# Tanveer81/ReVisionLLM

Hardware: AMD Instinct MI355X
Metric: video-segments/sec (whole node), stage-2 100-seg recursion, Vicuna-7B (higher is better)
Workload: dtype fp16

## Files before the change

revisionllm_amd/csrc/attention.hip:

```cpp
#include "kernels.h"

#ifndef ATTN_PAIR_Q32
#define ATTN_PAIR_Q32 0
#endif

namespace {

template <int DH, bool SPLIT, bool PAD, bool QS = false>
__device__ __forceinline__ void attn_body(const AttnArgs& a, int bx, int h, int b, [[maybe_unused]] float* merge = nullptr) {
    constexpr int NC = DH / 32, ND = DH / 16;
    const int lane = threadIdx.x & 63;
    const int wave = __builtin_amdgcn_readfirstlane(threadIdx.x >> 6);
    const int fr = lane & 15, g = lane >> 4;
    const int q0 = SPLIT ? bx * 16 : bx * 64 + wave * 16;
    if (q0 >= a.Lq) return;
    const int kb_ = b / a.kv_div;
    const int Lk = a.row_pos ? a.row_pos[b] + 1 : a.Lk;
    if (Lk <= 0 || (a.row_pos && Lk > a.Lk)) return;
    const int q_pos0 = a.row_pos ? Lk - a.Lq : a.q_pos0;

    const op16_t* qp = (const op16_t*)a.q + (int64_t)b * a.q_bs + (int64_t)min(q0 + fr, a.Lq - 1) * a.q_rs + h * DH + g * 8;
    op16x8 qf[NC];
#pragma unroll
    for (int c = 0; c < NC; ++c) qf[c] = *(const op16x8*)(qp + c * 32);
    op16x8 ql[QS ? NC : 1];
    if constexpr (QS) {
#pragma unroll
        for (int c = 0; c < NC; ++c) ql[c] = *(const op16x8*)(qp + a.q_lo + c * 32);
    }

    const op16_t* kbase = (const op16_t*)a.k + (int64_t)kb_ * a.k_bs + (int64_t)h * a.k_hs + g * 8;
    const op16_t* vbase = (const op16_t*)a.vt + (int64_t)kb_ * a.vt_bs + (int64_t)h * a.vt_hs + (int64_t)fr * a.vt_ds + g * a.vt_ks;
    int share_len = 0;
// ... 491 lines not shown
        const float alpha = __expf(m_run - m_use);
        float psum = 0.f;
        float p[8];
#pragma unroll
        for (int t = 0; t < 2; ++t)
#pragma unroll
            for (int r = 0; r < 4; ++r) {
                const float e = __expf(s[t][r] - m_use);
                p[t * 4 + r] = e;
                psum += e;
            }
        l_run = l_run * alpha + psum;
        m_run = m_new;
        union { op16x8 v; uint32_t u[4]; } pf;
#pragma unroll
        for (int j = 0; j < 4; ++j) pf.u[j] = pack_op16x2_bounded(p[2 * j], p[2 * j + 1]);
        if (__builtin_amdgcn_ballot_w64(alpha != 1.0f) != 0) {
#pragma unroll
            for (int dt = 0; dt < ND; ++dt) o[dt] *= alpha;
        }
#pragma unroll
        for (int dt = 0; dt < ND; ++dt) o[dt] = rv_mfma16(vf[dt], pf.v, o[dt]);
    }
    l_run += __shfl_xor(l_run, 16, 64);
    l_run += __shfl_xor(l_run, 32, 64);
    if (q0 + fr >= a.Lq) return;
    const float inv = 1.0f / l_run;
    op16_t* op = (op16_t*)a.out + (int64_t)b * a.o_bs + (int64_t)(q0 + fr) * a.o_rs + h * DH + g * 4;
#pragma unroll
    for (int dt = 0; dt < ND; ++dt)
        *(u32x2*)(op + dt * 16) = pack_op16x4(f32x4{o[dt][0] * inv, o[dt][1] * inv, o[dt][2] * inv, o[dt][3] * inv});
}

__device__ __forceinline__ bool attn_map(int tiles, int H, int pairs, int& bx, int& h, int& b) {
    const int id = blockIdx.x, j = id >> 3;
    const int pr = (j / tiles) * 8 + (id & 7);
    if (pr >= pairs) return false;
    bx = j % tiles;
    h = pr % H;
    b = pr / H;
    return true;
}
__host__ inline unsigned attn_grid(int tiles, int pairs) { return (unsigned)(tiles * ((pairs + 7) / 8) * 8); }

template <int DH, bool SPLIT, bool QS = false>
__global__ __launch_bounds__(256, DH <= 128 ? 3 : 1) void attn_kernel(AttnArgs a, int tiles) {
    int bx, h, b;
    if (!attn_map(tiles, a.H, a.H * a.B, bx, h, b)) return;
    __shared__ __attribute__((aligned(16))) float merge[SPLIT ? 4 * 16 * (DH + 4) + 2 * 4 * 16 : 4];
    if constexpr (QS) attn_body<DH, SPLIT, false, true>(a, bx, h, b, merge);
    else if (a.key_pad) attn_body<DH, SPLIT, true>(a, bx, h, b, merge);
    else attn_body<DH, SPLIT, false>(a, bx, h, b, merge);
}

template <int DH>
__global__ __launch_bounds__(256, 2) void attn_kernel_lds(AttnArgs a, int tiles) {
    __shared__ __attribute__((aligned(16))) char smem[2 * (2 * (DH / 32) + DH / 16) * 1024];
    int bx, h, b;
    if (!attn_map(tiles, a.H, a.H * a.B, bx, h, b)) return;
    attn_body_lds<DH>(a, bx, h, b, smem);
}

template <int DH, bool QS = false>
__global__ __launch_bounds__(256, 3) void attn_kernel_pair(AttnArgs a, AttnArgs b, int tiles, AttnGroups gr) {
    int bx, h, z;
    const int per = a.B + b.B;
// ... 44 lines not shown
}

__device__ __forceinline__ void attn_mixed_problem(AttnArgs& p, const AttnMixed& mx, int z, int& b) {
    int g = 0;
    for (int i = 1; i < mx.G; ++i) g += z >= mx.first[i] ? 1 : 0;
    const QkvGroup e = mx.gt[g];
    const int zl = z - mx.first[g], hasp = e.P0 > 0 ? 1 : 0;
    const bool prefix = hasp && zl == 0;
    const int64_t row0 = prefix ? e.base : e.base + e.P0;
    p.q = (const op16_t*)p.q + row0 * p.q_rs;
    p.out = (op16_t*)p.out + row0 * p.o_rs;
    p.k = (const op16_t*)p.k + (int64_t)e.row * p.k_bs;
    p.vt = (const op16_t*)p.vt + (int64_t)e.row * p.vt_bs;
    if (prefix) { p.B = 1; p.Lq = p.Lk = e.P0; p.q_pos0 = 0; p.q_bs = (int64_t)e.P0 * p.q_rs; p.o_bs = (int64_t)e.P0 * p.o_rs; b = 0; }
    else { p.B = e.B; p.Lq = e.S; p.Lk = e.P0 + e.S; p.q_pos0 = e.P0; p.q_bs = (int64_t)e.S * p.q_rs; p.o_bs = (int64_t)e.S * p.o_rs; b = zl - hasp; }
}
template <int DH>
__global__ __launch_bounds__(256, 2) void attn_kernel_mixed_lds(AttnArgs a, AttnMixed mx, int tiles) {
    __shared__ __attribute__((aligned(16))) char smem[2 * (2 * (DH / 32) + DH / 16) * 1024];
    int bx, h, z, b;
    if (!attn_map(tiles, a.H, a.H * mx.problems, bx, h, z)) return;
    attn_mixed_problem(a, mx, z, b);
    if (bx * 64 >= a.Lq) return;
    attn_body_lds1<DH>(a, bx, h, b, smem);
}
template <int DH>
__global__ __launch_bounds__(256, 3) void attn_kernel_mixed(AttnArgs a, AttnMixed mx, int tiles) {
    int bx, h, z, b;
    if (!attn_map(tiles, a.H, a.H * mx.problems, bx, h, z)) return;
    attn_mixed_problem(a, mx, z, b);
    if (bx * 64 >= a.Lq) return;
    attn_body<DH, false, false, false>(a, bx, h, b);
}
__global__ void mixed_tables_kernel(AttnMixed mx, QkvGroup* gt, int* last_rows) {
    if (threadIdx.x >= (unsigned)mx.G) return;
    const QkvGroup e = mx.gt[threadIdx.x];
    gt[threadIdx.x] = e;
    if (!last_rows) return;
    int o = 0;
    for (int i = 0; i < (int)threadIdx.x; ++i) o += mx.gt[i].B;
    for (int b = 0; b < e.B; ++b) last_rows[o + b] = e.base + e.P0 + (b + 1) * e.S - 1;
}

}

static int attn_check(const AttnArgs& a) {
    RV_CHECK_ARG(a.q && a.k && a.vt && a.out, "attention: null tensor");
    RV_CHECK_ARG(a.B > 0 && a.H > 0 && a.Lq > 0 && a.Lk > 0 && a.kv_div > 0, "attention: empty problem");
    RV_CHECK_ARG(a.q_rs % 8 == 0 && a.k_rs % 8 == 0 && a.k_hs % 8 == 0 && a.vt_ds % 8 == 0 && a.vt_hs % 8 == 0 && a.vt_bs % 8 == 0 && a.o_rs % 4 == 0,
                 "attention: stride alignment");
    RV_CHECK_ARG(a.vt_ks != 8 || a.vt_ds >= ((a.Lk + 31) / 32) * 32, "attention: V^T rows must be padded to a multiple of 32 keys");
    return RV_OK;
}

int k_attention_pair(const AttnArgs& a, const AttnArgs& b, hipStream_t st, const AttnGroups* groups) {
    if (int rc = attn_check(a)) return rc;
    if (int rc = attn_check(b)) return rc;
    RV_CHECK_ARG(a.dh == 128 && b.dh == 128 && a.H == b.H && a.Lq > 16 && b.Lq > 16, "attention pair: 128-wide heads, same head count, prefill lengths only");
    RV_CHECK_ARG(!a.key_pad && !b.key_pad, "attention pair: key padding is not supported");
    const int tiles = (int)cdiv(a.Lq > b.Lq ? a.Lq : b.Lq, (ATTN_PAIR_Q32 && !a.q_lo) ? 128 : 64);
    const AttnGroups gr = groups ? *groups : AttnGroups{};
    RV_CHECK_ARG(gr.G >= 1 && gr.G <= RV_MAX_PREFILL_GROUPS, "attention pair: 1 .. %d groups", RV_MAX_PREFILL_GROUPS);
    RV_CHECK_ARG((a.q_lo != 0) == (b.q_lo != 0), "attention pair: both problems or neither carry split queries");
    const bool lds = !a.q_lo && !ATTN_PAIR_Q32 && rv_cur_opts().attn_lds && !a.row_pos && !b.row_pos && !a.out_lo && !b.out_lo;
    if (a.q_lo) hipLaunchKernelGGL((attn_kernel_pair<128, true>), dim3(attn_grid(tiles, a.H * (a.B + b.B) * gr.G)), dim3(256), 0, st, a, b, tiles, gr);
    else if (lds) hipLaunchKernelGGL((attn_kernel_pair_lds<128>), dim3(attn_grid(tiles, a.H * (a.B + b.B) * gr.G)), dim3(256), 0, st, a, b, tiles, gr);
    else hipLaunchKernelGGL((attn_kernel_pair<128>), dim3(attn_grid(tiles, a.H * (a.B + b.B) * gr.G)), dim3(256), 0, st, a, b, tiles, gr);
    RV_CHECK_LAUNCH("attention pair");
    return RV_OK;
}

int k_attention_groups(const AttnArgs& b, hipStream_t st, const AttnGroups& gr) {
    if (int rc = attn_check(b)) return rc;
    RV_CHECK_ARG(b.dh == 128 && b.Lq > 16 && !b.key_pad && !b.row_pos, "attention groups: 128-wide heads, prefill lengths, no key padding, no per-row positions");
    RV_CHECK_ARG(gr.G >= 1 && gr.G <= RV_MAX_PREFILL_GROUPS, "attention groups: 1 .. %d groups", RV_MAX_PREFILL_GROUPS);
    AttnArgs a = b;
    a.B = 0;
    const int tiles = (int)cdiv(b.Lq, (ATTN_PAIR_Q32 && !b.q_lo) ? 128 : 64);
    const bool lds = !b.q_lo && !ATTN_PAIR_Q32 && rv_cur_opts().attn_lds && !b.out_lo;
    if (b.q_lo) hipLaunchKernelGGL((attn_kernel_pair<128, true>), dim3(attn_grid(tiles, b.H * b.B * gr.G)), dim3(256), 0, st, a, b, tiles, gr);
    else if (lds) hipLaunchKernelGGL((attn_kernel_pair_lds<128>), dim3(attn_grid(tiles, b.H * b.B * gr.G)), dim3(256), 0, st, a, b, tiles, gr);
    else hipLaunchKernelGGL((attn_kernel_pair<128>), dim3(attn_grid(tiles, b.H * b.B * gr.G)), dim3(256), 0, st, a, b, tiles, gr);
    RV_CHECK_LAUNCH("attention groups");
    return RV_OK;
}

int k_attention_mixed(const AttnArgs& a, const AttnMixed& mx, hipStream_t st) {
    RV_CHECK_ARG(a.q && a.k && a.vt && a.out, "attention mixed: null tensor");
    RV_CHECK_ARG(a.dh == 128 && a.H > 0 && !a.key_pad && !a.row_pos && !a.q_lo && !a.out_lo && a.causal && a.kv_div == 1,
                 "attention mixed: causal 128-wide heads, no key padding, no per-row positions, no split operands");
    RV_CHECK_ARG(a.q_rs % 8 == 0 && a.k_rs % 8 == 0 && a.k_hs % 8 == 0 && a.vt_ds % 8 == 0 && a.vt_hs % 8 == 0 && a.vt_bs % 8 == 0 && a.o_rs % 4 == 0,
                 "attention: stride alignment");
    RV_CHECK_ARG(mx.G >= 1 && mx.G <= RV_MAX_PREFILL_GROUPS, "attention mixed: 1 .. %d groups", RV_MAX_PREFILL_GROUPS);
    int longest = 0, problems = 0;
    for (int g = 0; g < mx.G; ++g) {
        const QkvGroup& e = mx.gt[g];
        RV_CHECK_ARG(e.B > 0 && e.S > 16 && (e.P0 == 0 || e.P0 > 16) && e.row >= 0 && e.base >= 0, "attention mixed: group %d: prefill lengths only (S > 16, P0 == 0 or > 16)", g);
        RV_CHECK_ARG(a.vt_ks != 8 || a.vt_ds >= ((e.P0 + e.S + 31) / 32) * 32, "attention: V^T rows must be padded to a multiple of 32 keys");
        RV_CHECK_ARG(mx.first[g] == problems, "attention mixed: group %d: first problem %d, expected %d", g, mx.first[g], problems);
        problems += (e.P0 > 0 ? 1 : 0) + e.B;
        longest = e.S > longest ? e.S : longest;
        longest = e.P0 > longest ? e.P0 : longest;
    }
    RV_CHECK_ARG(mx.problems == problems, "attention mixed: %d problems, expected %d", mx.problems, problems);
    const int tiles = (int)cdiv(longest, 64);
    const dim3 grid(attn_grid(tiles, a.H * problems));
    if (rv_cur_opts().attn_lds) hipLaunchKernelGGL((attn_kernel_mixed_lds<128>), grid, dim3(256), 0, st, a, mx, tiles);
    else hipLaunchKernelGGL((attn_kernel_mixed<128>), grid, dim3(256), 0, st, a, mx, tiles);
    RV_CHECK_LAUNCH("attention mixed");
    return RV_OK;
}

int k_mixed_tables(const AttnMixed& mx, QkvGroup* gt, int* last_rows, hipStream_t st) {
    RV_CHECK_ARG(gt && mx.G >= 1 && mx.G <= RV_MAX_PREFILL_GROUPS, "mixed tables: bad argument");
    hipLaunchKernelGGL(mixed_tables_kernel, dim3(1), dim3(64), 0, st, mx, gt, last_rows);
    RV_CHECK_LAUNCH("mixed tables");
    return RV_OK;
}

int k_attention(const AttnArgs& a, hipStream_t st) {
    RV_CHECK_ARG(a.q && a.k && a.vt && a.out, "attention: null tensor");
    RV_CHECK_ARG(a.B > 0 && a.H > 0 && a.Lq > 0 && a.Lk > 0 && a.kv_div > 0, "attention: empty problem");
    RV_CHECK_ARG(a.q_rs % 8 == 0 && a.k_rs % 8 == 0 && a.k_hs % 8 == 0 && a.vt_ds % 8 == 0 && a.vt_hs % 8 == 0 && a.vt_bs % 8 == 0 && a.o_rs % 4 == 0,
                 "attention: stride alignment");
    RV_CHECK_ARG(a.vt_ks != 8 || a.vt_ds >= ((a.Lk + 31) / 32) * 32, "attention: V^T rows must be padded to a multiple of 32 keys");
    const bool split = a.Lq <= 16 && !a.no_split;
    const int tiles = (int)cdiv(a.Lq, split ? 16 : 64);
    const dim3 grid(attn_grid(tiles, a.H * a.B));
    if (a.q_lo) {
        RV_CHECK_ARG(a.dh == 128 && !a.key_pad, "attention: split queries are instantiated for 128-wide heads without key padding");
        if (split) hipLaunchKernelGGL((attn_kernel<128, true, true>), grid, dim3(256), 0, st, a, tiles);
        else hipLaunchKernelGGL((attn_kernel<128, false, true>), grid, dim3(256), 0, st, a, tiles);
        RV_CHECK_LAUNCH("attention");
        return RV_OK;
    }
    const bool lds = !split && !a.key_pad && !a.causal && !a.row_pos && !a.row_share && !a.out_packed && !a.out_lo && a.Lk >= 96 && a.Lq >= 48 &&
                     (a.dh == 64 || a.dh == 96) && rv_cur_opts().attn_lds;
    if (lds) {
        const int t128 = (int)cdiv(a.Lq, 128);
        const dim3 g128(attn_grid(t128, a.H * a.B));
        if (a.dh == 64) hipLaunchKernelGGL((attn_kernel_lds<64>), g128, dim3(256), 0, st, a, t128);
        else hipLaunchKernelGGL((attn_kernel_lds<96>), g128, dim3(256), 0, st, a, t128);
        RV_CHECK_LAUNCH("attention (LDS-staged keys)");
        return RV_OK;
    }
    if (!split && a.dh == 128 && !a.key_pad && !a.row_pos && !a.row_share && !a.out_packed && !a.out_lo && a.Lk >= 64 && a.Lq > 16 && rv_cur_opts().attn_lds) {
        hipLaunchKernelGGL((attn_kernel_lds1<128>), grid, dim3(256), 0, st, a, tiles);
        RV_CHECK_LAUNCH("attention (LDS-staged keys, dh 128)");
        return RV_OK;
    }
    if (a.dh == 64 && !split)
        hipLaunchKernelGGL((attn_kernel<64, false>), grid, dim3(256), 0, st, a, tiles);
    else if (a.dh == 64)
        hipLaunchKernelGGL((attn_kernel<64, true>), grid, dim3(256), 0, st, a, tiles);
    else if (a.dh == 96 && !split)
        hipLaunchKernelGGL((attn_kernel<96, false>), grid, dim3(256), 0, st, a, tiles);
    else if (a.dh == 96)
        hipLaunchKernelGGL((attn_kernel<96, true>), grid, dim3(256), 0, st, a, tiles);
    else if (a.dh == 128 && !split)
        hipLaunchKernelGGL((attn_kernel<128, false>), grid, dim3(256), 0, st, a, tiles);
    else if (a.dh == 128)
        hipLaunchKernelGGL((attn_kernel<128, true>), grid, dim3(256), 0, st, a, tiles);
    else if (a.dh == 512) {
        const int t512 = (int)cdiv(a.Lq, 64);
        hipLaunchKernelGGL((attn_kernel<512, false>), dim3(attn_grid(t512, a.H * a.B)), dim3(256), 0, st, a, t512);
    }
    else {
        rv_set_error("attention: head dim %d unsupported (64, 96, 128)", a.dh);
        return RV_ERR_ARG;
    }
    RV_CHECK_LAUNCH("attention");
    return RV_OK;
}

extern "C" int rv_attention(const void* q, int64_t q_row_stride, int64_t q_batch_stride, const void* k, int64_t k_row_stride,
                            int64_t k_batch_stride, int64_t k_head_stride, const void* vt, int64_t vt_batch_stride,
                            int64_t vt_head_stride, int64_t vt_d_stride, void* out, int64_t o_row_stride, int64_t o_batch_stride,
                            const uint8_t* key_pad, int32_t B, int32_t H, int32_t dh, int32_t Lq, int32_t Lk, int32_t causal,
                            int32_t q_pos0, int32_t kv_batch_div, float scale, void* stream) {
// ... 8 lines not shown
```

revisionllm_amd/csrc/engine.hip:

```cpp
#include <string>
#include <unordered_map>
#include <vector>

#include "kernels.h"

struct Tensor {
    const void* p = nullptr;
    int dtype = 0;
    int64_t numel = 0;
};

struct AdapterLayer {
    const op16_t *w_in, *w_out, *w1, *w2;
    const float *b_in, *b_out, *b1, *b2, *ln1_w, *ln1_b, *ln2_w, *ln2_b;
};
struct LlmLayer {
    const op16_t *wqkv, *wo, *wgu, *wdown;
    const float *norm1, *norm2;
    const uint8_t *wqkv8 = nullptr, *wo8 = nullptr, *wgu8 = nullptr, *wdown8 = nullptr;
    const float *sqkv = nullptr, *so = nullptr, *sgu = nullptr, *sdown = nullptr;
    const uint8_t *wqkv8p = nullptr, *wo8p = nullptr, *wgu8p = nullptr, *wdown8p = nullptr;
    const op16_t *wqkv2 = nullptr, *wo2 = nullptr, *wgu2 = nullptr, *wdown2 = nullptr;
};

// ... 264 lines not shown
    if (k == "sample_variant") return &o.sample_variant;
    if (k == "gemm_arows") return &o.gemm_arows;
    if (k == "rows_fill") return &o.rows_fill;
    if (k == "rows_spread") return &o.rows_spread;
    if (k == "rows_persistent") return &o.rows_persistent;
    if (k == "rows_single") return &o.rows_single;
    if (k == "gemm_waves") return &o.gemm_waves;
    if (k == "gemm_mhalf") return &o.gemm_mhalf;
    if (k == "precision") return &o.precision;
    if (k == "lm_head_split") return &o.lm_head_split;
    if (k == "last_block_rows") return &o.last_block_rows;
    if (k == "adapter_stream16") return &o.adapter_stream16;
    if (k == "adapter_fold_t2v") return &o.adapter_fold_t2v;
    if (k == "attn_lds") return &o.attn_lds;
    if (k == "qkv_lds") return &o.qkv_lds;
    return nullptr;
}
}

unsigned int* rv_numeric_bound();

extern "C" int rv_ctx_set_option(rv_ctx* c, const char* key, int64_t value) {
    RV_CHECK_ARG(c && key, "rv_ctx_set_option: null argument");
    if (std::string(key) == "saturated") {
        RV_CHECK_ARG(value == 0, "rv_ctx_set_option: 'saturated' can only be reset to 0");
        if (unsigned int* p = rv_numeric_bound()) {
            if (hipDeviceSynchronize() != hipSuccess || hipMemset(p, 0, 16) != hipSuccess) {
                rv_set_error("rv_ctx_set_option: resetting the numeric status failed: %s", hipGetErrorString(hipGetLastError()));
                return RV_ERR_HIP;
            }
        }
        return RV_OK;
    }
    int* slot = option_slot(c->opt, key);
    RV_CHECK_ARG(slot, "rv_ctx_set_option: unknown option '%s'", key);
    const std::string k(key);
    if (k == "gemm_tile_variant") RV_CHECK_ARG(value >= 0 && value <= 6, "rv_ctx_set_option: gemm_tile_variant must be in [0, 6]");
    if (k == "gemm_waves") RV_CHECK_ARG(value == 4 || value == 8, "rv_ctx_set_option: gemm_waves must be 4 or 8");
    if (k == "gemm_cus") RV_CHECK_ARG(value >= 0 && value % 8 == 0, "rv_ctx_set_option: gemm_cus must be a non-negative multiple of 8");
    if (k == "precision") RV_CHECK_ARG(value == 0 || value == 1, "rv_ctx_set_option: precision must be 0 (bf16 operands) or 1 (parity: split operands)");
    *slot = (int)value;
    return RV_OK;
}

extern "C" int rv_ctx_get_option(const rv_ctx* c, const char* key, int64_t* value) {
    RV_CHECK_ARG(c && key && value, "rv_ctx_get_option: null argument");
    if (std::string(key) == "saturated") {
        *value = 0;
        if (unsigned int* p = rv_numeric_bound()) {
            unsigned int n = 0;
            if (hipDeviceSynchronize() != hipSuccess || hipMemcpy(&n, p, sizeof(n), hipMemcpyDeviceToHost) != hipSuccess) {
                rv_set_error("rv_ctx_get_option: reading the numeric status failed: %s", hipGetErrorString(hipGetLastError()));
                return RV_ERR_HIP;
            }
            *value = n;
        }
        return RV_OK;
    }
    const int* slot = option_slot(const_cast<rv_ctx*>(c)->opt, key);
    RV_CHECK_ARG(slot, "rv_ctx_get_option: unknown option '%s'", key);
    *value = *slot;
    return RV_OK;
}

extern "C" int rv_weights_bind(rv_ctx* c, const char* name, const void* dptr, int dtype, int64_t numel) {
    RV_CHECK_ARG(c && name && dptr && numel > 0, "rv_weights_bind: bad arguments");
    RV_CHECK_ARG(!c->options_only, "rv_weights_bind: this context was created without a model configuration");
    RV_CHECK_ARG(((uintptr_t)dptr & 15) == 0, "rv_weights_bind: '%s' must be 16-byte aligned", name);
    c->w[name] = Tensor{dptr, dtype, numel};
    c->resolved_adapter = c->resolved_llm = c->resolved_proj = false;
    return RV_OK;
}

extern "C" int rv_project_dense(rv_ctx* c, const void* x_bf16, void* y, int out_dtype, int64_t rows, void* stream) {
    RV_CHECK_ARG(c && x_bf16 && y && rows > 0, "rv_project_dense: bad arguments");
    RvOptScope scope(&c->opt);
    RV_TRY(resolve_proj(c));
    const int64_t d = c->cfg.adapter_dim, D = c->cfg.hidden;
    return rv_gemm_impl(x_bf16, d, c->proj_w, d, 1, c->proj_b, nullptr, 0, y, D, out_dtype, RV_ACT_NONE, rows, D, d, nullptr, 0, as_stream(stream));
}

extern "C" size_t rv_clip_encoder_ws_bytes(const rv_ctx* c, int32_t N, int32_t T, int32_t Nq, int32_t Lq) {
    if (!c || N <= 0 || T <= 0) return 0;
    return carve_clip(c, nullptr, 0, N, T, Nq, Lq).bytes;
}

extern "C" int rv_clip_encoder(rv_ctx* c, const void* x, const void* txt, const uint8_t* txt_mask, int32_t N, int32_t T,
                               int32_t Nq, int32_t Lq, int32_t feature, float* out, void* ws, size_t ws_bytes, void* stream) {
    RV_CHECK_ARG(c && x && out && ws, "rv_clip_encoder: null argument");
// ... 83 lines not shown
                    RV_TRY(k_layernorm(nullptr, L.ln2_w, L.ln2_b, nullptr, w.x16, w.xp16, w.pm + d, T, R0, (int)d, st, T, ys16));
                    RV_TRY(k_cls_rows(c->cls_token, w.pm, nullptr, w.x16, w.xp16, N, T, (int)d, st));
                }
                continue;
            }
            if (!fold)
                RV_TRY(rv_gemm_impl(w.a16, d, L.w_out, d, 1, L.b_out, v32, d, w.y32, d, RV_F32, RV_ACT_NONE, R0, d, d, w.sk, w.sk_bytes, st));
            RV_TRY(k_layernorm(w.y32, L.ln1_w, L.ln1_b, nullptr, w.x16, nullptr, nullptr, 0, R0, (int)d, st));
            RV_TRY(rv_gemm_impl(w.x16, d, L.w1, d, 1, L.b1, nullptr, 0, w.h16, ff, RV_OP16, RV_ACT_RELU, R0, ff, d, w.sk, w.sk_bytes, st));
            RV_TRY(rv_gemm_impl(w.h16, ff, L.w2, ff, 1, L.b2, w.y32, d, w.y32, d, RV_F32, RV_ACT_NONE, R0, d, ff, w.sk, w.sk_bytes, st));
            if (l + 1 < c->t2v.size()) {
                RV_TRY(k_layernorm(w.y32, L.ln2_w, L.ln2_b, v32, nullptr, vp16, w.pm + d, T, R0, (int)d, st));
            } else {
                RV_TRY(k_layernorm(w.y32, L.ln2_w, L.ln2_b, w.x32, w.x16, w.xp16, w.pm + d, T, R0, (int)d, st, T));
                RV_TRY(k_cls_rows(c->cls_token, w.pm, w.x32, w.x16, w.xp16, N, T, (int)d, st));
            }
        }
    } else {
        RV_TRY(k_build_x(x, nullptr, c->cls_token, w.pm, s16 ? nullptr : w.x32, w.x16, w.xp16, N, T, (int)d, st));
    }

    for (size_t l = 0; l < c->enc.size(); ++l) {
        const AdapterLayer& L = c->enc[l];
        if (feature == RV_FEAT_CLS && l + 1 == c->enc.size() && N > 16 && T >= 3) {
            const int64_t sx = (int64_t)(T + 1) * d;
            op16_t* kk16 = w.qk16;
            op16_t* qc16 = w.h16;
            float* y0 = w.y32;
            float* y1 = w.y32 + (int64_t)N * d;
            float* y2 = w.y32 + (int64_t)2 * N * d;
            RV_TRY(rv_gemm_impl(w.xp16, d, L.w_in + d * d, d, 1, L.b_in + d, nullptr, 0, kk16, d, RV_OP16, RV_ACT_NONE, R1, d, d, w.sk, w.sk_bytes, st));
            RV_TRY(rv_gemm_impl(w.xp16, sx, L.w_in, d, 1, L.b_in, nullptr, 0, qc16, d, RV_OP16, RV_ACT_NONE, N, d, d, w.sk, w.sk_bytes, st, nullptr, 0, 1));
            RV_TRY(rv_gemm_impl(w.x16, d, L.w_in + 2 * d * d, d, 1, L.b_in + 2 * d, nullptr, 0, w.vv16, d, RV_OP16, RV_ACT_NONE, R1, d, d, w.sk, w.sk_bytes, st));
            RV_TRY(k_transpose_v(w.vv16, d, w.vt16, N, T + 1, w.Lpad, H, dh, st));
            AttnArgs a{qc16, d, d, kk16, d, (int64_t)(T + 1) * d, dh, w.vt16, (int64_t)d * w.Lpad, (int64_t)dh * w.Lpad, w.Lpad, w.a16, d, d,
                       nullptr, N, H, dh, 1, T + 1, 0, 0, 1, scale, 1};
            RV_TRY(k_attention(a, st));
            const float* cls_res = w.x32;
            int64_t cls_ld = sx;
            if (s16) {
                float* y3 = w.y32 + (int64_t)3 * N * d;
                RV_TRY(k_rows_to_f32(w.x16, sx, y3, N, (int)d, st));
                cls_res = y3;
                cls_ld = d;
            }
            RV_TRY(rv_gemm_impl(w.a16, d, L.w_out, d, 1, L.b_out, cls_res, cls_ld, y0, d, RV_F32, RV_ACT_NONE, N, d, d, w.sk, w.sk_bytes, st, nullptr, 0, 1));
            RV_TRY(k_layernorm(y0, L.ln1_w, L.ln1_b, y1, w.x16, nullptr, nullptr, 0, N, (int)d, st, 0, nullptr, s16 ? 3 : 0));
            RV_TRY(rv_gemm_impl(w.x16, d, L.w1, d, 1, L.b1, nullptr, 0, w.h16, ff, RV_OP16, RV_ACT_RELU, N, ff, d, w.sk, w.sk_bytes, st, nullptr, 0, 1));
            RV_TRY(rv_gemm_impl(w.h16, ff, L.w2, ff, 1, L.b2, y1, d, y2, d, RV_F32, RV_ACT_NONE, N, d, ff, w.sk, w.sk_bytes, st, nullptr, 0, 1));
            if (!c->adp_proj_w)
                return k_layernorm(y2, L.ln2_w, L.ln2_b, (float*)out, nullptr, nullptr, nullptr, 0, N, (int)d, st);
            RV_TRY(k_layernorm(y2, L.ln2_w, L.ln2_b, nullptr, w.x16, nullptr, nullptr, 0, N, (int)d, st, 0, nullptr, s16 ? 1 : 0));
            return rv_gemm_impl(w.x16, d, c->adp_proj_w, d, 1, c->adp_proj_b, nullptr, 0, out, D, RV_F32, RV_ACT_NONE, N, D, d, w.sk, w.sk_bytes, st, nullptr, 0, 1);
        }
        RV_TRY(rv_gemm_impl(w.xp16, d, L.w_in, d, 1, L.b_in, nullptr, 0, w.qk16, 2 * d, RV_OP16, RV_ACT_NONE, R1, 2 * d, d, w.sk, w.sk_bytes, st));
        RV_TRY(rv_gemm_impl(w.x16, d, L.w_in + 2 * d * d, d, 1, L.b_in + 2 * d, nullptr, 0, w.vv16, d, RV_OP16, RV_ACT_NONE, R1, d, d, w.sk, w.sk_bytes, st));
        RV_TRY(k_transpose_v(w.vv16, d, w.vt16, N, T + 1, w.Lpad, H, dh, st));
        AttnArgs a{w.qk16, 2 * d, (int64_t)(T + 1) * 2 * d, w.qk16 + d, 2 * d, (int64_t)(T + 1) * 2 * d, dh, w.vt16,
                   (int64_t)d * w.Lpad, (int64_t)dh * w.Lpad, w.Lpad, w.a16, d, (int64_t)(T + 1) * d, nullptr, N, H, dh, T + 1,
                   T + 1, 0, 0, 1, scale};
        RV_TRY(k_attention(a, st));
        if (s16) {
            RV_TRY(rv_gemm_impl(w.a16, d, L.w_out, d, 1, L.b_out, (const float*)w.x16, d, ys16, d, RV_OP16, RV_ACT_NONE, R1, d, d, w.sk, w.sk_bytes, st, nullptr, 1));
            RV_TRY(k_layernorm(nullptr, L.ln1_w, L.ln1_b, nullptr, w.x16, nullptr, nullptr, 0, R1, (int)d, st, 0, ys16));
            RV_TRY(rv_gemm_impl(w.x16, d, L.w1, d, 1, L.b1, nullptr, 0, w.h16, ff, RV_OP16, RV_ACT_RELU, R1, ff, d, w.sk, w.sk_bytes, st));
            RV_TRY(rv_gemm_impl(w.h16, ff, L.w2, ff, 1, L.b2, (const float*)w.x16, d, ys16, d, RV_OP16, RV_ACT_NONE, R1, d, ff, w.sk, w.sk_bytes, st, nullptr, 1));
            RV_TRY(k_layernorm(nullptr, L.ln2_w, L.ln2_b, nullptr, w.x16, w.xp16, w.pm, T + 1, R1, (int)d, st, 0, ys16));
            continue;
        }
        RV_TRY(rv_gemm_impl(w.a16, d, L.w_out, d, 1, L.b_out, w.x32, d, w.y32, d, RV_F32, RV_ACT_NONE, R1, d, d, w.sk, w.sk_bytes, st));
        RV_TRY(k_layernorm(w.y32, L.ln1_w, L.ln1_b, w.x32, w.x16, nullptr, nullptr, 0, R1, (int)d, st));
        RV_TRY(rv_gemm_impl(w.x16, d, L.w1, d, 1, L.b1, nullptr, 0, w.h16, ff, RV_OP16, RV_ACT_RELU, R1, ff, d, w.sk, w.sk_bytes, st));
        RV_TRY(rv_gemm_impl(w.h16, ff, L.w2, ff, 1, L.b2, w.x32, d, w.y32, d, RV_F32, RV_ACT_NONE, R1, d, ff, w.sk, w.sk_bytes, st));
        RV_TRY(k_layernorm(w.y32, L.ln2_w, L.ln2_b, w.x32, w.x16, w.xp16, w.pm, T + 1, R1, (int)d, st));
    }
    if (!c->adp_proj_w) {
        const hipError_t e = feature == RV_FEAT_CLS
                                 ? hipMemcpy2DAsync(out, (size_t)d * 4, w.x32, (size_t)(T + 1) * d * 4, (size_t)d * 4, (size_t)N, hipMemcpyDeviceToDevice, st)
                                 : hipMemcpyAsync(out, w.x32, (size_t)R1 * d * 4, hipMemcpyDeviceToDevice, st);
        if (e != hipSuccess) {
            rv_set_error("rv_clip_encoder: output copy failed: %s", hipGetErrorString(e));
            return RV_ERR_HIP;
        }
        return RV_OK;
    }
    if (feature == RV_FEAT_CLS)
        return rv_gemm_impl(w.x16, (int64_t)(T + 1) * d, c->adp_proj_w, d, 1, c->adp_proj_b, nullptr, 0, out, D, RV_F32, RV_ACT_NONE, N, D,
                            d, w.sk, w.sk_bytes, st);
    return rv_gemm_impl(w.x16, d, c->adp_proj_w, d, 1, c->adp_proj_b, nullptr, 0, out, D, RV_F32, RV_ACT_NONE, R1, D, d, w.sk, w.sk_bytes, st);
}

extern "C" int rv_splice_embed(rv_ctx* c, const int32_t* map, const float* video_rows, float* h, int64_t rows, void* stream) {
    RV_CHECK_ARG(c && map && h && rows > 0, "rv_splice_embed: bad arguments");
// ... 487 lines not shown
```

revisionllm_amd/csrc/kernels.h:

```cpp
#pragma once
#include "common.h"

struct RvOpts {
    int gemm_tile_variant = 2;
    int gemm_cus = 0;
    int fp8_decode = 1;
    int fp8_prefill = 1;
    int sample_variant = 1;
    int gemm_arows = 1;
    int gemm_waves = 8;
    int gemm_mhalf = 2;
    int rows_single = 1;
    int rows_persistent = 1;
    int rows_spread = 0;
    int rows_fill = 240;
    int lm_head_split = 1;
    int last_block_rows = 1;
    int adapter_stream16 = 1;
    int adapter_fold_t2v = 1;
    int attn_lds = 1;
    int qkv_lds = 1;
    int precision = 0;
};
extern const RvOpts g_default_opts;
// ... 186 lines not shown
int k_split_bf16(const float* x, int64_t ldx, void* y16, int64_t rows, int n, hipStream_t st);
int k_qkv_rope_split(const float* qkv32, int64_t ld, const QkvRope& qr, int64_t M, int64_t D, hipStream_t st);
int k_gather_last_rows(const void* a16, const float* h, const int* idx, int64_t rows, int Mg, int P0, int B, int S, void* a_out, float* h_out, int D, hipStream_t st);
int k_t2v_fold(const void* wq_p, const float* bq, const void* wo_p, const void* tk16, const void* tv16, int64_t ld, int Nq, int Lq, int LK, int H, int dh, float scale,
               void* A1p, float* c1, void* A2p, hipStream_t st);
int k_t2v_softmax(const float* S, const uint8_t* pad, void* P16, int64_t rows, int H, int LK, int Lq, int64_t rows_per_query, hipStream_t st);
int k_sine_pos(float* pos, int T, int d, hipStream_t st);
int k_frames_in(const void* x16, const float* pos, float* v32, void* vp16, int64_t rows, int T, int d, hipStream_t st);
int k_build_x(const void* src16, const float* src32, const float* cls, const float* pm, float* x32, void* x16, void* xp16,
              int64_t N, int T, int d, hipStream_t st);
int k_copy_f32(const float* src, float* dst, int64_t n, hipStream_t st);
int k_rows_to_f32(const void* src16, int64_t ld, float* dst, int64_t rows, int d, hipStream_t st);
int k_cls_rows(const float* cls, const float* pm, float* x32, void* x16, void* xp16, int64_t N, int T, int d, hipStream_t st);
int k_transpose_v(const void* v, int64_t ld, void* vt, int64_t Nb, int L, int Lpad, int H, int dh, hipStream_t st);
int k_rope_table(float* cs, int S, int pos0, int dh, float theta, hipStream_t st);
int k_rope_table_rows(float* cs, const int* row_pos, int rows, int dh, float theta, hipStream_t st);
int k_splice_embed(const int32_t* map, const void* embed, const float* video, float* h, int64_t rows, int D, hipStream_t st);

struct AttnArgs {
    const void* q; int64_t q_rs, q_bs;
    const void* k; int64_t k_rs, k_bs, k_hs;
    const void* vt; int64_t vt_bs, vt_hs, vt_ds;
    void* out; int64_t o_rs, o_bs;
    const uint8_t* key_pad;
    int B, H, dh, Lq, Lk, causal, q_pos0, kv_div;
    float scale;
    int no_split = 0;
    const int* row_pos = nullptr;
    int out_packed = 0;
    int64_t vt_ks = 8;
    int64_t out_lo = 0;
    int64_t q_lo = 0;
    const int* row_share = nullptr;
};
int k_attention(const AttnArgs& a, hipStream_t st);
struct AttnGroups {
    int G = 1;
    int64_t q_off[RV_MAX_PREFILL_GROUPS] = {0, 0, 0, 0, 0, 0, 0, 0};
    int64_t o_off[RV_MAX_PREFILL_GROUPS] = {0, 0, 0, 0, 0, 0, 0, 0};
    int64_t kv_off[RV_MAX_PREFILL_GROUPS] = {0, 0, 0, 0, 0, 0, 0, 0};
};
int k_attention_pair(const AttnArgs& a, const AttnArgs& b, hipStream_t st, const AttnGroups* groups = nullptr);
int k_attention_groups(const AttnArgs& a, hipStream_t st, const AttnGroups& groups);
struct AttnMixed {
    int G = 0, problems = 0;
    int first[RV_MAX_PREFILL_GROUPS] = {};
    QkvGroup gt[RV_MAX_PREFILL_GROUPS] = {};
};
int k_attention_mixed(const AttnArgs& a, const AttnMixed& mx, hipStream_t st);
int k_mixed_tables(const AttnMixed& mx, QkvGroup* gt, int* last_rows, hipStream_t st);
```

Baseline: 6438.

## Add resident-key attention kernels staging all K/V in LDS per head

Adds attention kernels in which one workgroup per (batch, head) stages every key/value fragment into up to 160 KB of dynamic LDS once, then loops its waves over all query tiles. This removes the repeated per-tile global loads of K and V. For the adapter's dh-96 layers it also reads row-major V straight from LDS with transposing LDS reads, so the separate V-transpose kernel can be skipped. The path is on by default only for dh 96 (attn_lds=1), while the dh-128 LLM paths need attn_lds=3. The cost is lower occupancy, because each block holds a large LDS allocation, and fewer blocks when there are few heads.

```diff
diff --git a/revisionllm_amd/csrc/attention.hip b/revisionllm_amd/csrc/attention.hip
--- a/revisionllm_amd/csrc/attention.hip
+++ b/revisionllm_amd/csrc/attention.hip
@@ -1,4 +1,5 @@
 #include "kernels.h"
+#include <atomic>
 
 #ifndef ATTN_PAIR_Q32
 #define ATTN_PAIR_Q32 0
@@ -556,6 +557,170 @@
         *(u32x2*)(op + dt * 16) = pack_op16x4(f32x4{o[dt][0] * inv, o[dt][1] * inv, o[dt][2] * inv, o[dt][3] * inv});
 }
 
+constexpr int ATTN_RES_WAVES = 9;
+constexpr int ATTN_RES_LDS = 160 * 1024;
+template <int DH>
+__host__ __device__ constexpr int attn_res_stage() { return (2 * (DH / 32) + DH / 16) * 1024; }
+template <int DH>
+__host__ inline bool attn_res_fits(int keys, int queries) {
+    return (int64_t)((keys + 31) / 32) * attn_res_stage<DH>() <= ATTN_RES_LDS && queries <= 4 * ATTN_RES_WAVES * 16;
+}
+extern __shared__ __attribute__((aligned(16))) char attn_res_smem[];
+
+typedef __attribute__((ext_vector_type(4))) short attn_i16x4;
+__device__ __forceinline__ uint32_t attn_res_pack_p(float lo, float hi) {
+#if RV_OP_F16
+    uint32_t w;
+    asm("s_nop 0\n\tv_cvt_pk_f16_f32 %0, %1, %2" : "=v"(w) : "v"(lo), "v"(hi));
+    return w;
+#else
+    return pack_op16x2_bounded(lo, hi);
+#endif
+}
+template <int DH, bool VROWS = false>
+__device__ __forceinline__ void attn_body_res(const AttnArgs& a, int h, int b, char* smem) {
+    constexpr int NC = DH / 32, ND = DH / 16, NF = 2 * NC + ND;
+    const int lane = threadIdx.x & 63;
+    const int wave = __builtin_amdgcn_readfirstlane(threadIdx.x >> 6);
+    const int waves = (int)(blockDim.x >> 6);
+    const int fr = lane & 15, g = lane >> 4;
+    const int kb_ = b / a.kv_div;
+    const int Lk = a.Lk, q_pos0 = a.q_pos0;
+    const op16_t* kbase = (const op16_t*)a.k + (int64_t)kb_ * a.k_bs + (int64_t)h * a.k_hs + g * 8;
+    const op16_t* vbase = (const op16_t*)a.vt + (int64_t)kb_ * a.vt_bs + (int64_t)h * a.vt_hs + (int64_t)fr * a.vt_ds + g * a.vt_ks;
+    const int krow = (fr >> 2) * 8 + (fr & 3);
+    const op16_t* vrows = VROWS ? (const op16_t*)a.v_rows + (int64_t)kb_ * a.v_bs + h * DH : nullptr;
+    const int kend_wg = a.causal ? min(Lk, q_pos0 + a.Lq) : Lk;
+    const int nfrag = ((kend_wg + 31) >> 5) * NF;
+    for (int F = wave; F < nfrag; F += waves) {
+        const int blk = F / NF, f = F - blk * NF, k0 = blk * 32;
+        const op16_t* src;
+        if (f < 2 * NC) {
+            const int t = f / NC, c = f - t * NC;
+            src = kbase + (int64_t)min(k0 + krow + t * 4, Lk - 1) * a.k_rs + c * 32;
+        } else if constexpr (VROWS) {
+            const int ci = (f - 2 * NC) * 64 + lane, row = ci / (DH / 8), ch = ci - row * (DH / 8);
+            src = vrows + (int64_t)min(k0 + row, Lk - 1) * a.v_rs + ch * 8;
+        } else {
+            src = vbase + (int64_t)(f - 2 * NC) * 16 * a.vt_ds + (int64_t)(k0 >> 3) * a.vt_ks;
+        }
+        __builtin_amdgcn_global_load_lds((attn_gptr_t)src, (attn_lptr_t)(smem + (int64_t)F * 1024), 16, 0, 0);
+    }
+    const int ntiles = (a.Lq + 15) >> 4;
+    bool staged = false;
+    for (int pass = 0;; ++pass) {
+        const int tile = (pass & 1) ? (pass + 1) * waves - 1 - wave : pass * waves + wave;
+        if (pass * waves >= ntiles) break;
+        const bool active = tile < ntiles;
+        const int q0 = tile * 16;
+        op16x8 qf[NC];
+        if (active) {
+            const op16_t* qp = (const op16_t*)a.q + (int64_t)b * a.q_bs + (int64_t)min(q0 + fr, a.Lq - 1) * a.q_rs + h * DH + g * 8;
+#pragma unroll
+            for (int c = 0; c < NC; ++c) qf[c] = *(const op16x8*)(qp + c * 32);
+        }
+        if (!staged) {
+            asm volatile("s_waitcnt vmcnt(0)" ::: "memory");
+            __builtin_amdgcn_s_barrier();
+            asm volatile("" ::: "memory");
+            staged = true;
+        }
+        if (!active) continue;
+        f32x4 o[ND];
+#pragma unroll
+        for (int i = 0; i < ND; ++i) o[i] = f32x4{0.f, 0.f, 0.f, 0.f};
+        float m_run = -INFINITY, l_run = 0.f;
+        const int qpos = q_pos0 + q0 + fr;
+        const int kend = a.causal ? min(Lk, q_pos0 + min(q0 + 16, a.Lq)) : Lk;
+        for (int k0 = 0; k0 < kend; k0 += 32) {
+            const char* buf = smem + (k0 >> 5) * (NF * 1024) + lane * 16;
+            op16x8 kf[2][NC];
+#pragma unroll
+            for (int t = 0; t < 2; ++t)
+#pragma unroll
+                for (int c = 0; c < NC; ++c) kf[t][c] = *(const op16x8*)(buf + (t * NC + c) * 1024);
+            op16x8 vf[ND];
+            if constexpr (VROWS) {
+                const char* vimg = smem + (k0 >> 5) * (NF * 1024) + 2 * NC * 1024 + ((8 * g + (fr >> 2)) * DH + (fr & 3) * 4) * 2;
+#pragma unroll
+                for (int dt = 0; dt < ND; ++dt) {
+                    union { op16x8 v; attn_i16x4 h[2]; } u;
+                    u.h[0] = __builtin_amdgcn_ds_read_tr16_b64_v4i16((__attribute__((address_space(3))) attn_i16x4*)(vimg + dt * 32));
+                    u.h[1] = __builtin_amdgcn_ds_read_tr16_b64_v4i16((__attribute__((address_space(3))) attn_i16x4*)(vimg + 4 * DH * 2 + dt * 32));
+                    vf[dt] = u.v;
+                }
+            } else {
+#pragma unroll
+                for (int dt = 0; dt < ND; ++dt) vf[dt] = *(const op16x8*)(buf + (2 * NC + dt) * 1024);
+            }
+            f32x4 s[2];
+#pragma unroll
+            for (int t = 0; t < 2; ++t) {
+                s[t] = f32x4{0.f, 0.f, 0.f, 0.f};
+#pragma unroll
+                for (int c = 0; c < NC; ++c) s[t] = rv_mfma16(kf[t][c], qf[c], s[t]);
+            }
+            float mx = -INFINITY;
+            const bool interior = k0 + 32 <= Lk && (!a.causal || k0 + 31 <= q_pos0 + q0);
+            if (interior) {
+#pragma unroll
+                for (int t = 0; t < 2; ++t)
+#pragma unroll
+                    for (int r = 0; r < 4; ++r) {
+                        s[t][r] *= a.scale;
+                        mx = fmaxf(mx, s[t][r]);
+                    }
+            } else {
+#pragma unroll
+                for (int t = 0; t < 2; ++t)
+#pragma unroll
+                    for (int r = 0; r < 4; ++r) {
+                        const int key = k0 + g * 8 + t * 4 + r;
+                        const bool dead = key >= Lk || (a.causal && key > qpos);
+                        const float v = dead ? -INFINITY : s[t][r] * a.scale;
+                        s[t][r] = v;
+                        mx = fmaxf(mx, v);
+                    }
+            }
+            mx = fmaxf(mx, __shfl_xor(mx, 16, 64));
+            mx = fmaxf(mx, __shfl_xor(mx, 32, 64));
+            const float m_new = fmaxf(m_run, mx);
+            const float m_use = m_new == -INFINITY ? 0.f : m_new;
+            const float alpha = __expf(m_run - m_use);
+            float psum = 0.f;
+            float p[8];
+#pragma unroll
+            for (int t = 0; t < 2; ++t)
+#pragma unroll
+                for (int r = 0; r < 4; ++r) {
+                    const float e = __expf(s[t][r] - m_use);
+                    p[t * 4 + r] = e;
+                    psum += e;
+                }
+            l_run = l_run * alpha + psum;
+            m_run = m_new;
+            union { op16x8 v; uint32_t u[4]; } pf;
+#pragma unroll
+            for (int j = 0; j < 4; ++j) pf.u[j] = attn_res_pack_p(p[2 * j], p[2 * j + 1]);
+            if (__builtin_amdgcn_ballot_w64(alpha != 1.0f) != 0) {
+#pragma unroll
+                for (int dt = 0; dt < ND; ++dt) o[dt] *= alpha;
+            }
+#pragma unroll
+            for (int dt = 0; dt < ND; ++dt) o[dt] = rv_mfma16(vf[dt], pf.v, o[dt]);
+        }
+        l_run += __shfl_xor(l_run, 16, 64);
+        l_run += __shfl_xor(l_run, 32, 64);
+        if (q0 + fr < a.Lq) {
+            const float inv = 1.0f / l_run;
+            op16_t* op = (op16_t*)a.out + (int64_t)b * a.o_bs + (int64_t)(q0 + fr) * a.o_rs + h * DH + g * 4;
+#pragma unroll
+            for (int dt = 0; dt < ND; ++dt)
+                *(u32x2*)(op + dt * 16) = pack_op16x4(f32x4{o[dt][0] * inv, o[dt][1] * inv, o[dt][2] * inv, o[dt][3] * inv});
+        }
+    }
+}
+
 __device__ __forceinline__ bool attn_map(int tiles, int H, int pairs, int& bx, int& h, int& b) {
     const int id = blockIdx.x, j = id >> 3;
     const int pr = (j / tiles) * 8 + (id & 7);
@@ -666,6 +831,35 @@
     if (bx * 64 >= a.Lq) return;
     attn_body<DH, false, false, false>(a, bx, h, b);
 }
+template <int DH, bool VROWS = false>
+__global__ __launch_bounds__(ATTN_RES_WAVES * 64) void attn_kernel_res(AttnArgs a) {
+    int bx, h, b;
+    if (!attn_map(1, a.H, a.H * a.B, bx, h, b)) return;
+    attn_body_res<DH, VROWS>(a, h, b, attn_res_smem);
+}
+template <int DH>
+__global__ __launch_bounds__(ATTN_RES_WAVES * 64) void attn_kernel_pair_res(AttnArgs a, AttnArgs b, AttnGroups gr) {
+    int bx, h, z;
+    const int per = a.B + b.B;
+    if (!attn_map(1, a.H, a.H * per * gr.G, bx, h, z)) return;
+    const int g = z / per;
+    z -= g * per;
+    AttnArgs& p = z < a.B ? a : b;
+    if (gr.G > 1) {
+        p.q = (const op16_t*)p.q + gr.q_off[g];
+        p.out = (op16_t*)p.out + gr.o_off[g];
+        p.k = (const op16_t*)p.k + gr.kv_off[g];
+        p.vt = (const op16_t*)p.vt + gr.kv_off[g];
+    }
+    attn_body_res<DH>(p, h, z < a.B ? z : z - a.B, attn_res_smem);
+}
+template <int DH>
+__global__ __launch_bounds__(ATTN_RES_WAVES * 64) void attn_kernel_mixed_res(AttnArgs a, AttnMixed mx) {
+    int bx, h, z, b;
+    if (!attn_map(1, a.H, a.H * mx.problems, bx, h, z)) return;
+    attn_mixed_problem(a, mx, z, b);
+    attn_body_res<DH>(a, h, b, attn_res_smem);
+}
 __global__ void mixed_tables_kernel(AttnMixed mx, QkvGroup* gt, int* last_rows) {
     if (threadIdx.x >= (unsigned)mx.G) return;
     const QkvGroup e = mx.gt[threadIdx.x];
@@ -684,6 +878,25 @@
     RV_CHECK_ARG(a.q_rs % 8 == 0 && a.k_rs % 8 == 0 && a.k_hs % 8 == 0 && a.vt_ds % 8 == 0 && a.vt_hs % 8 == 0 && a.vt_bs % 8 == 0 && a.o_rs % 4 == 0,
                  "attention: stride alignment");
     RV_CHECK_ARG(a.vt_ks != 8 || a.vt_ds >= ((a.Lk + 31) / 32) * 32, "attention: V^T rows must be padded to a multiple of 32 keys");
+    return RV_OK;
+}
+
+static std::atomic<long long> g_attn_resident_launches{0};
+long long rv_attn_resident_launches() { return g_attn_resident_launches.load(std::memory_order_relaxed); }
+
+template <int DH, class Kern, class... Args>
+static int attn_res_launch(Kern kern, const char* what, int pairs, int longest_q, int longest_k, hipStream_t st, Args... args) {
+    const int tiles = (longest_q + 15) / 16;
+    const int waves = tiles < 4 ? 4 : tiles < ATTN_RES_WAVES ? tiles : ATTN_RES_WAVES;
+    const unsigned threads = 64u * (unsigned)waves;
+    const size_t lds = (size_t)((longest_k + 31) / 32) * attn_res_stage<DH>();
+    if (hipFuncSetAttribute((const void*)kern, hipFuncAttributeMaxDynamicSharedMemorySize, ATTN_RES_LDS) != hipSuccess) {
+        rv_set_error("%s: raising the kernel's LDS limit failed: %s", what, hipGetErrorString(hipGetLastError()));
+        return RV_ERR_HIP;
+    }
+    hipLaunchKernelGGL(kern, dim3(attn_grid(1, pairs)), dim3(threads), lds, st, args...);
+    RV_CHECK_LAUNCH(what);
+    g_attn_resident_launches.fetch_add(1, std::memory_order_relaxed);
     return RV_OK;
 }
 
@@ -697,6 +910,9 @@
     RV_CHECK_ARG(gr.G >= 1 && gr.G <= RV_MAX_PREFILL_GROUPS, "attention pair: 1 .. %d groups", RV_MAX_PREFILL_GROUPS);
     RV_CHECK_ARG((a.q_lo != 0) == (b.q_lo != 0), "attention pair: both problems or neither carry split queries");
     const bool lds = !a.q_lo && !ATTN_PAIR_Q32 && rv_cur_opts().attn_lds && !a.row_pos && !b.row_pos && !a.out_lo && !b.out_lo;
+    if (lds && rv_cur_opts().attn_lds == 3 && attn_res_fits<128>(a.Lk > b.Lk ? a.Lk : b.Lk, a.Lq > b.Lq ? a.Lq : b.Lq))
+        return attn_res_launch<128>(attn_kernel_pair_res<128>, "attention pair (resident keys)", a.H * (a.B + b.B) * gr.G, a.Lq > b.Lq ? a.Lq : b.Lq,
+                                    a.Lk > b.Lk ? a.Lk : b.Lk, st, a, b, gr);
     if (a.q_lo) hipLaunchKernelGGL((attn_kernel_pair<128, true>), dim3(attn_grid(tiles, a.H * (a.B + b.B) * gr.G)), dim3(256), 0, st, a, b, tiles, gr);
     else if (lds) hipLaunchKernelGGL((attn_kernel_pair_lds<128>), dim3(attn_grid(tiles, a.H * (a.B + b.B) * gr.G)), dim3(256), 0, st, a, b, tiles, gr);
     else hipLaunchKernelGGL((attn_kernel_pair<128>), dim3(attn_grid(tiles, a.H * (a.B + b.B) * gr.G)), dim3(256), 0, st, a, b, tiles, gr);
@@ -712,6 +928,8 @@
     a.B = 0;
     const int tiles = (int)cdiv(b.Lq, (ATTN_PAIR_Q32 && !b.q_lo) ? 128 : 64);
     const bool lds = !b.q_lo && !ATTN_PAIR_Q32 && rv_cur_opts().attn_lds && !b.out_lo;
+    if (lds && rv_cur_opts().attn_lds == 3 && attn_res_fits<128>(b.Lk, b.Lq))
+        return attn_res_launch<128>(attn_kernel_pair_res<128>, "attention groups (resident keys)", b.H * b.B * gr.G, b.Lq, b.Lk, st, a, b, gr);
     if (b.q_lo) hipLaunchKernelGGL((attn_kernel_pair<128, true>), dim3(attn_grid(tiles, b.H * b.B * gr.G)), dim3(256), 0, st, a, b, tiles, gr);
     else if (lds) hipLaunchKernelGGL((attn_kernel_pair_lds<128>), dim3(attn_grid(tiles, b.H * b.B * gr.G)), dim3(256), 0, st, a, b, tiles, gr);
     else hipLaunchKernelGGL((attn_kernel_pair<128>), dim3(attn_grid(tiles, b.H * b.B * gr.G)), dim3(256), 0, st, a, b, tiles, gr);
@@ -726,7 +944,7 @@
     RV_CHECK_ARG(a.q_rs % 8 == 0 && a.k_rs % 8 == 0 && a.k_hs % 8 == 0 && a.vt_ds % 8 == 0 && a.vt_hs % 8 == 0 && a.vt_bs % 8 == 0 && a.o_rs % 4 == 0,
                  "attention: stride alignment");
     RV_CHECK_ARG(mx.G >= 1 && mx.G <= RV_MAX_PREFILL_GROUPS, "attention mixed: 1 .. %d groups", RV_MAX_PREFILL_GROUPS);
-    int longest = 0, problems = 0;
+    int longest = 0, longest_k = 0, problems = 0;
     for (int g = 0; g < mx.G; ++g) {
         const QkvGroup& e = mx.gt[g];
         RV_CHECK_ARG(e.B > 0 && e.S > 16 && (e.P0 == 0 || e.P0 > 16) && e.row >= 0 && e.base >= 0, "attention mixed: group %d: prefill lengths only (S > 16, P0 == 0 or > 16)", g);
@@ -735,8 +953,11 @@
         problems += (e.P0 > 0 ? 1 : 0) + e.B;
         longest = e.S > longest ? e.S : longest;
         longest = e.P0 > longest ? e.P0 : longest;
+        longest_k = e.P0 + e.S > longest_k ? e.P0 + e.S : longest_k;
     }
     RV_CHECK_ARG(mx.problems == problems, "attention mixed: %d problems, expected %d", mx.problems, problems);
+    if (rv_cur_opts().attn_lds == 3 && attn_res_fits<128>(longest_k, longest))
+        return attn_res_launch<128>(attn_kernel_mixed_res<128>, "attention mixed (resident keys)", a.H * problems, longest, longest_k, st, a, mx);
     const int tiles = (int)cdiv(longest, 64);
     const dim3 grid(attn_grid(tiles, a.H * problems));
     if (rv_cur_opts().attn_lds) hipLaunchKernelGGL((attn_kernel_mixed_lds<128>), grid, dim3(256), 0, st, a, mx, tiles);
@@ -752,8 +973,16 @@
     return RV_OK;
 }
 
+static bool attn_res96(const AttnArgs& a) {
+    const bool split = a.Lq <= 16 && !a.no_split;
+    return !split && !a.q_lo && !a.key_pad && !a.causal && !a.row_pos && !a.row_share && !a.out_packed && !a.out_lo && a.dh == 96 && a.Lk >= 96 &&
+           (a.Lq >= 48 || a.v_rows) && (rv_cur_opts().attn_lds == 1 || rv_cur_opts().attn_lds == 3) && attn_res_fits<96>(a.Lk, a.Lq);
+}
+bool k_attention_reads_v_rows(const AttnArgs& a) { return a.v_rows && attn_res96(a); }
+
 int k_attention(const AttnArgs& a, hipStream_t st) {
     RV_CHECK_ARG(a.q && a.k && a.vt && a.out, "attention: null tensor");
+    RV_CHECK_ARG(!a.v_rows || (a.v_rs % 8 == 0 && a.v_bs % 8 == 0 && ((uintptr_t)a.v_rows & 15) == 0), "attention: row-major V: stride / pointer alignment");
     RV_CHECK_ARG(a.B > 0 && a.H > 0 && a.Lq > 0 && a.Lk > 0 && a.kv_div > 0, "attention: empty problem");
     RV_CHECK_ARG(a.q_rs % 8 == 0 && a.k_rs % 8 == 0 && a.k_hs % 8 == 0 && a.vt_ds % 8 == 0 && a.vt_hs % 8 == 0 && a.vt_bs % 8 == 0 && a.o_rs % 4 == 0,
                  "attention: stride alignment");
@@ -770,6 +999,10 @@
     }
     const bool lds = !split && !a.key_pad && !a.causal && !a.row_pos && !a.row_share && !a.out_packed && !a.out_lo && a.Lk >= 96 && a.Lq >= 48 &&
                      (a.dh == 64 || a.dh == 96) && rv_cur_opts().attn_lds;
+    if (attn_res96(a)) {
+        if (a.v_rows) return attn_res_launch<96>(attn_kernel_res<96, true>, "attention (resident keys, row-major V)", a.H * a.B, a.Lq, a.Lk, st, a);
+        return attn_res_launch<96>(attn_kernel_res<96>, "attention (resident keys)", a.H * a.B, a.Lq, a.Lk, st, a);
+    }
     if (lds) {
         const int t128 = (int)cdiv(a.Lq, 128);
         const dim3 g128(attn_grid(t128, a.H * a.B));
@@ -779,6 +1012,8 @@
         return RV_OK;
     }
     if (!split && a.dh == 128 && !a.key_pad && !a.row_pos && !a.row_share && !a.out_packed && !a.out_lo && a.Lk >= 64 && a.Lq > 16 && rv_cur_opts().attn_lds) {
+        if (rv_cur_opts().attn_lds == 3 && attn_res_fits<128>(a.Lk, a.Lq))
+            return attn_res_launch<128>(attn_kernel_res<128>, "attention (resident keys, dh 128)", a.H * a.B, a.Lq, a.Lk, st, a);
         hipLaunchKernelGGL((attn_kernel_lds1<128>), grid, dim3(256), 0, st, a, tiles);
         RV_CHECK_LAUNCH("attention (LDS-staged keys, dh 128)");
         return RV_OK;
diff --git a/revisionllm_amd/csrc/engine.hip b/revisionllm_amd/csrc/engine.hip
--- a/revisionllm_amd/csrc/engine.hip
+++ b/revisionllm_amd/csrc/engine.hip
@@ -320,12 +320,14 @@
         }
         return RV_OK;
     }
+    RV_CHECK_ARG(std::string(key) != "attn_resident_launches", "rv_ctx_set_option: 'attn_resident_launches' is a read-only counter");
     int* slot = option_slot(c->opt, key);
     RV_CHECK_ARG(slot, "rv_ctx_set_option: unknown option '%s'", key);
     const std::string k(key);
     if (k == "gemm_tile_variant") RV_CHECK_ARG(value >= 0 && value <= 6, "rv_ctx_set_option: gemm_tile_variant must be in [0, 6]");
     if (k == "gemm_waves") RV_CHECK_ARG(value == 4 || value == 8, "rv_ctx_set_option: gemm_waves must be 4 or 8");
     if (k == "gemm_cus") RV_CHECK_ARG(value >= 0 && value % 8 == 0, "rv_ctx_set_option: gemm_cus must be a non-negative multiple of 8");
+    if (k == "attn_lds") RV_CHECK_ARG(value >= 0 && value <= 3, "rv_ctx_set_option: attn_lds must be 0 (per wave), 1 (resident adapter layers, staged otherwise), 2 (staged) or 3 (resident wherever it fits)");
     if (k == "precision") RV_CHECK_ARG(value == 0 || value == 1, "rv_ctx_set_option: precision must be 0 (bf16 operands) or 1 (parity: split operands)");
     *slot = (int)value;
     return RV_OK;
@@ -343,6 +345,10 @@
             }
             *value = n;
         }
+        return RV_OK;
+    }
+    if (std::string(key) == "attn_resident_launches") {
+        *value = rv_attn_resident_launches();
         return RV_OK;
     }
     const int* slot = option_slot(const_cast<rv_ctx*>(c)->opt, key);
@@ -492,9 +498,12 @@
             RV_TRY(rv_gemm_impl(w.xp16, d, L.w_in + d * d, d, 1, L.b_in + d, nullptr, 0, kk16, d, RV_OP16, RV_ACT_NONE, R1, d, d, w.sk, w.sk_bytes, st));
             RV_TRY(rv_gemm_impl(w.xp16, sx, L.w_in, d, 1, L.b_in, nullptr, 0, qc16, d, RV_OP16, RV_ACT_NONE, N, d, d, w.sk, w.sk_bytes, st, nullptr, 0, 1));
             RV_TRY(rv_gemm_impl(w.x16, d, L.w_in + 2 * d * d, d, 1, L.b_in + 2 * d, nullptr, 0, w.vv16, d, RV_OP16, RV_ACT_NONE, R1, d, d, w.sk, w.sk_bytes, st));
-            RV_TRY(k_transpose_v(w.vv16, d, w.vt16, N, T + 1, w.Lpad, H, dh, st));
             AttnArgs a{qc16, d, d, kk16, d, (int64_t)(T + 1) * d, dh, w.vt16, (int64_t)d * w.Lpad, (int64_t)dh * w.Lpad, w.Lpad, w.a16, d, d,
                        nullptr, N, H, dh, 1, T + 1, 0, 0, 1, scale, 1};
+            a.v_rows = w.vv16;
+            a.v_rs = d;
+            a.v_bs = (int64_t)(T + 1) * d;
+            if (!k_attention_reads_v_rows(a)) RV_TRY(k_transpose_v(w.vv16, d, w.vt16, N, T + 1, w.Lpad, H, dh, st));
             RV_TRY(k_attention(a, st));
             const float* cls_res = w.x32;
             int64_t cls_ld = sx;
@@ -515,10 +524,13 @@
         }
         RV_TRY(rv_gemm_impl(w.xp16, d, L.w_in, d, 1, L.b_in, nullptr, 0, w.qk16, 2 * d, RV_OP16, RV_ACT_NONE, R1, 2 * d, d, w.sk, w.sk_bytes, st));
         RV_TRY(rv_gemm_impl(w.x16, d, L.w_in + 2 * d * d, d, 1, L.b_in + 2 * d, nullptr, 0, w.vv16, d, RV_OP16, RV_ACT_NONE, R1, d, d, w.sk, w.sk_bytes, st));
-        RV_TRY(k_transpose_v(w.vv16, d, w.vt16, N, T + 1, w.Lpad, H, dh, st));
         AttnArgs a{w.qk16, 2 * d, (int64_t)(T + 1) * 2 * d, w.qk16 + d, 2 * d, (int64_t)(T + 1) * 2 * d, dh, w.vt16,
                    (int64_t)d * w.Lpad, (int64_t)dh * w.Lpad, w.Lpad, w.a16, d, (int64_t)(T + 1) * d, nullptr, N, H, dh, T + 1,
                    T + 1, 0, 0, 1, scale};
+        a.v_rows = w.vv16;
+        a.v_rs = d;
+        a.v_bs = (int64_t)(T + 1) * d;
+        if (!k_attention_reads_v_rows(a)) RV_TRY(k_transpose_v(w.vv16, d, w.vt16, N, T + 1, w.Lpad, H, dh, st));
         RV_TRY(k_attention(a, st));
         if (s16) {
             RV_TRY(rv_gemm_impl(w.a16, d, L.w_out, d, 1, L.b_out, (const float*)w.x16, d, ys16, d, RV_OP16, RV_ACT_NONE, R1, d, d, w.sk, w.sk_bytes, st, nullptr, 1));
diff --git a/revisionllm_amd/csrc/kernels.h b/revisionllm_amd/csrc/kernels.h
--- a/revisionllm_amd/csrc/kernels.h
+++ b/revisionllm_amd/csrc/kernels.h
@@ -242,8 +242,12 @@
     int64_t out_lo = 0;
     int64_t q_lo = 0;
     const int* row_share = nullptr;
-};
+    const void* v_rows = nullptr;
+    int64_t v_rs = 0, v_bs = 0;
+};
+bool k_attention_reads_v_rows(const AttnArgs& a);
 int k_attention(const AttnArgs& a, hipStream_t st);
+long long rv_attn_resident_launches();
 struct AttnGroups {
     int G = 1;
     int64_t q_off[RV_MAX_PREFILL_GROUPS] = {0, 0, 0, 0, 0, 0, 0, 0};
```

Result: no change. 6416 (median of 2 runs) (-0.3%).
